# jean-pierreBoth/hnswlib-rs

Hardware: AMD Instinct MI355X
Metric: queries/sec (+ recall@10), batched HNSW search (higher is better)
Workload: dtype f32

## Files before the change

hnswlib-rs_amd/csrc/search_device.hip:

```cpp
#include <hip/hip_runtime.h>

#include <algorithm>
#include <chrono>
#include <cmath>
#include <cstdio>
#include <cstdlib>
#include <cstring>
#include <thread>
#include <vector>

#include "hnswio.hpp"
#include "search_device.hpp"
#include "search_kernels.hpp"
#include "worker_pool.hpp"

namespace hnswgpu {

namespace {
Knobs read_knobs() {
    Knobs k;
    auto num = [](const char* name, int unset) { const char* e = std::getenv(name); return e ? std::atoi(e) : unset; };
    auto flag = [](const char* name) { return std::getenv(name) != nullptr; };
    k.hash_bits = num("HNSWGPU_HASH_BITS", -1);
    k.no_sched = flag("HNSWGPU_NO_SCHED");
    k.no_pair_descent = flag("HNSWGPU_NO_PAIR_DESCENT");
    k.no_inkernel = flag("HNSWGPU_NO_INKERNEL");
    k.strict_wg_per_cu = num("HNSWGPU_STRICT_WG_PER_CU", -1);
    k.cand_lds = num("HNSWGPU_CAND_LDS", -1);
    k.waves_per_cu = num("HNSWGPU_WAVES_PER_CU", -1);
    k.exact_first = num("HNSWGPU_EXACT_FIRST", -1);
    k.trace_launch = flag("HNSWGPU_TRACE_LAUNCH");
    k.trace_host = flag("HNSWGPU_TRACE_HOST");
    k.host_threads = num("HNSWGPU_HOST_THREADS", -1);
    k.host_chunks = num("HNSWGPU_HOST_CHUNKS", -1);
    k.ffi_unpack = flag("HNSWGPU_FFI_UNPACK");
    k.pair_search = num("HNSWGPU_PAIR_SEARCH", -1);
    k.pair_tbits_delta = num("HNSWGPU_PAIR_TBITS_DELTA", 0);
    k.pair_wg_per_cu = num("HNSWGPU_PAIR_WG_PER_CU", -1);
    return k;
}
std::atomic<const Knobs*> g_knobs{nullptr};
}
const Knobs& knobs() {
    const Knobs* k = g_knobs.load(std::memory_order_acquire);
    if (k == nullptr) {
        const Knobs* fresh = new Knobs(read_knobs());
        if (g_knobs.compare_exchange_strong(k, fresh, std::memory_order_acq_rel)) k = fresh;
        else delete fresh;
    }
    return *k;
}
void reload_knobs() {
    g_knobs.store(new Knobs(read_knobs()), std::memory_order_release);
}

namespace {

#define HIP_TRY(expr)                                                                          \
    do {                                                                                       \
        hipError_t e_ = (expr);                                                                \
        if (e_ != hipSuccess) {                                                                \
            err = std::string(#expr) + ": " + hipGetErrorString(e_);                           \
            return ERR_DEVICE;                                                                 \
        }                                                                                      \
    } while (0)

hipError_t wait_stream(hipStream_t s) {
    const auto t0 = std::chrono::steady_clock::now();
    for (;;) {
        const hipError_t e = hipStreamQuery(s);
        if (e != hipErrorNotReady) return e;
        if (std::chrono::steady_clock::now() - t0 > std::chrono::milliseconds(20)) return hipStreamSynchronize(s);
    }
}
hipError_t wait_event(hipEvent_t ev) {
    const auto t0 = std::chrono::steady_clock::now();
    for (;;) {
        const hipError_t e = hipEventQuery(ev);
        if (e != hipErrorNotReady) return e;
        if (std::chrono::steady_clock::now() - t0 > std::chrono::milliseconds(20)) return hipEventSynchronize(ev);
    }
}

class DeviceGuard {
public:
    explicit DeviceGuard(int device) {
        if (device < 0) return;
        int cur = -1;
        if (hipGetDevice(&cur) != hipSuccess) cur = -1;
        if (cur == device) return;
        status_ = hipSetDevice(device);
        if (status_ == hipSuccess && cur >= 0) prev_ = cur;
    }
    ~DeviceGuard() { if (prev_ >= 0) (void)hipSetDevice(prev_); }
    DeviceGuard(const DeviceGuard&) = delete;
    DeviceGuard& operator=(const DeviceGuard&) = delete;
    hipError_t status() const { return status_; }
private:
    int prev_ = -1;
    hipError_t status_ = hipSuccess;
};

constexpr uint64_t PAIR_SEARCH_AUTO_MIN_QUERIES = 40000;
constexpr int STRICT_WG_PER_CU = 16;

uint32_t ceil_log2(uint64_t x) {
    uint32_t b = 0;
    while ((1ull << b) < x) ++b;
    return b;
}

const KernelSet& kernel_set(int metric) {
    switch (metric) {
        case DIST_L2: return kernels_for<DIST_L2>();
        case DIST_COSINE: return kernels_for<DIST_COSINE>();
        case DIST_DOT: return kernels_for<DIST_DOT>();
        case DIST_HELLINGER: return kernels_for<DIST_HELLINGER>();
        case DIST_JEFFREYS: return kernels_for<DIST_JEFFREYS>();
        case DIST_JENSENSHANNON: return kernels_for<DIST_JENSENSHANNON>();
        case KM_L2_SIMD8: return kernels_for<KM_L2_SIMD8>();
        case KM_COSINE_SIMD8: return kernels_for<KM_COSINE_SIMD8>();
        case KM_DOT_SIMD8: return kernels_for<KM_DOT_SIMD8>();
        case KM_L1_SIMD8: return kernels_for<KM_L1_SIMD8>();
        default: return kernels_for<DIST_L1>();
    }
}
// ... 50 lines not shown
    void free() {
        if (p) (void)hipHostFree(p);
        p = nullptr;
        dev = nullptr;
        cap = 0;
    }
};

void* pinned_alloc(size_t bytes, void** dev) {
    void* p = nullptr;
    if (hipHostMalloc(&p, bytes, hipHostMallocMapped | hipHostMallocPortable) != hipSuccess) { (void)hipGetLastError(); return nullptr; }
    if (hipHostGetDevicePointer(dev, p, 0) != hipSuccess) { (void)hipGetLastError(); (void)hipHostFree(p); return nullptr; }
    return p;
}
void pinned_free(void* p) {
    if (p) (void)hipHostFree(p);
}

struct DeviceIndex::Workspace {
    DevBuf qpad, tie, pre, order, retry[2], stats, bitmap, heaps, cand, oplog, allow, allowed_ids;
    PinnedBuf pin_in, pin_out;
    void* d_ctrl = nullptr;
    void* h_ctrl = nullptr;
    hipEvent_t ev_start = nullptr, ev_stop = nullptr, ev_ks = nullptr, ev_ke = nullptr;
    hipStream_t own_stream = nullptr;
    int init(std::string& err) {
        HIP_TRY(hipMalloc(&d_ctrl, 64));
        HIP_TRY(hipHostMalloc(&h_ctrl, 64, hipHostMallocDefault));
        HIP_TRY(hipEventCreate(&ev_start));
        HIP_TRY(hipEventCreate(&ev_stop));
        HIP_TRY(hipEventCreate(&ev_ks));
        HIP_TRY(hipEventCreate(&ev_ke));
        HIP_TRY(hipStreamCreateWithFlags(&own_stream, hipStreamNonBlocking));
        return OK;
    }
    ~Workspace() {
        for (DevBuf* b : {&qpad, &tie, &pre, &order, &retry[0], &retry[1], &stats, &bitmap, &heaps, &cand, &oplog, &allow, &allowed_ids})
            b->free();
        pin_in.free();
        pin_out.free();
        if (d_ctrl) (void)hipFree(d_ctrl);
        if (h_ctrl) (void)hipHostFree(h_ctrl);
        for (hipEvent_t e : {ev_start, ev_stop, ev_ks, ev_ke})
            if (e) (void)hipEventDestroy(e);
        if (own_stream) (void)hipStreamDestroy(own_stream);
    }
};

class DeviceIndex::Lease {
public:
    Lease(DeviceIndex* o, Workspace* w) : o_(o), w_(w) {}
    ~Lease() { if (w_) o_->release_ws(w_); }
    Lease(const Lease&) = delete;
    Lease& operator=(const Lease&) = delete;
    Workspace* get() const { return w_; }
private:
    DeviceIndex* o_;
    Workspace* w_;
};

DeviceIndex::Workspace* DeviceIndex::acquire(std::string& err) {
    {
        std::lock_guard<std::mutex> g(pool_mu_);
        if (!free_ws_.empty()) {
            Workspace* w = free_ws_.back();
// ... 132 lines not shown
CallInfo DeviceIndex::last_call() const {
    std::lock_guard<std::mutex> g(meta_mu_);
    return last_;
}

int DeviceIndex::upload(const FlatIndex& x, int device, std::string& err) {
    if (const char* e = std::getenv("HNSWGPU_STRICT_TIES")) strict_ties_.store(std::atoi(e) != 0);
    if (x.n == 0 || x.entry_flat == NO_POINT) { err = "cannot upload an empty index"; return ERR_EMPTY; }
    if (x.n >= 0x80000000ull) { err = "index too large for the device path (2^31 points or more)"; return ERR_ARG; }
    int ndev = 0;
    if (hipGetDeviceCount(&ndev) != hipSuccess || ndev == 0) { err = "no HIP device visible (a gfx950 GPU is required; there is no CPU fallback)"; return ERR_DEVICE; }
    if (device < 0 || device >= ndev) { err = "bad device ordinal"; return ERR_ARG; }
    release();
    DeviceGuard on_device(device);
    HIP_TRY(on_device.status());
    hipDeviceProp_t prop;
    HIP_TRY(hipGetDeviceProperties(&prop, device));
    num_cu_ = prop.multiProcessorCount;
    device_ = device;
    dist_ = x.dist;
    bytes_ = 0;
    descend_per_cu_[0].store(0);
    descend_per_cu_[1].store(0);

    const uint64_t n = x.n, d = x.dimension;
    DeviceIndexView v{};
    v.n = (uint32_t)n;
    v.d = (uint32_t)d;
    v.row_stride = (uint32_t)((d + 31) / 32 * 32);
    v.entry = x.entry_flat;
    v.entry_level = x.layer_of(x.entry_flat);
    v.search_layer = x.layer_to_search();
    for (unsigned l = 0; l <= NB_LAYER_MAX; ++l) v.layer_offset[l] = (uint32_t)x.layer_offset[l];

    {
        std::vector<float> pad((size_t)n * v.row_stride, 0.f);
        for (uint64_t f = 0; f < n; ++f) std::memcpy(pad.data() + f * v.row_stride, x.vectors.data() + f * d, d * sizeof(float));
        HIP_TRY(hipMalloc(&d_vec_, pad.size() * sizeof(float)));
        HIP_TRY(hipMemcpy(d_vec_, pad.data(), pad.size() * sizeof(float), hipMemcpyHostToDevice));
        bytes_ += pad.size() * sizeof(float);
    }
    {
        const unsigned sl = v.search_layer;
        uint64_t maxdeg = 1;
        for (uint64_t f = 0; f < n; ++f)
            maxdeg = std::max<uint64_t>(maxdeg, x.nbr_ptr[f * NB_LAYER_MAX + sl + 1] - x.nbr_ptr[f * NB_LAYER_MAX + sl]);
// ... 118 lines not shown
        a.id_stride = layout.id_stride;
        a.dist_stride = layout.dist_stride;
        a.count_stride = layout.count_stride;
        a.stats = stats;
        a.pre = w.pre.as<PreDescent>();
        x.heaps = w.heaps.as<hent_t>();
        x.heap_stride = heap_stride;
        x.cand_cap = (uint32_t)std::min<uint64_t>(cand_cap, 0xFFFFFFFFull);
        x.allow = d_allow;
        HIP_TRY(hipMemsetAsync(w.d_ctrl, 0, 16, stream));
        HIP_TRY(ks.launch_exact(ns, grid, lds, stream, v_, a, x));
        volatile uint32_t* ctrl = static_cast<volatile uint32_t*>(w.h_ctrl);
        HIP_TRY(hipMemcpyAsync(w.h_ctrl, w.d_ctrl, 16, hipMemcpyDeviceToHost, stream));
        HIP_TRY(wait_stream(stream));
        if (ctrl[1] != 0) { err = "internal error in the literal search kernel (a refused point inside return_points, or a candidate heap beyond every point)"; return ERR_DEVICE; }
        panics_total += ctrl[2];
        work = ctrl[3];
        qlist = w.retry[0].as<uint32_t>();
    }
    if (panics) *panics = panics_total;
    return OK;
}

int DeviceIndex::search_device(const float* d_queries, uint64_t nq, uint64_t d, uint64_t k, uint64_t ef_arg,
                               uint64_t* d_out_ids, float* d_out_dists, uint8_t* d_out_layer, int32_t* d_out_rank,
                               uint32_t* d_out_counts, uint32_t* d_stats, void* stream_v, const uint64_t* d_allowed,
                               uint64_t n_allowed, CallInfo* info_out, std::string& err, const RowFeed* feed, OutLayout layout) {
    if (!ready_) { err = "index is not resident on a device: call hnswgpu_upload first"; return ERR_DEVICE; }
    if (d != v_.d) { err = "query dimension differs from the index dimension"; return ERR_ARG; }
    CallInfo info{};
    auto publish = [&]() {
        if (info_out) *info_out = info;
        std::lock_guard<std::mutex> g(meta_mu_);
        last_ = info;
    };
    if (nq == 0) { publish(); return OK; }
    if (!d_queries || !d_out_ids || !d_out_dists || !d_out_counts) { err = "null buffer"; return ERR_ARG; }
    if (k == 0) { err = "knbn must be > 0"; return ERR_ARG; }
    const uint64_t ef = std::max(ef_arg, k);
    if (ef > 0x7FFFFFF0ull) { err = "ef too large"; return ERR_ARG; }
    if (nq > 0xFFFFFFF0ull) { err = "too many queries in one batch"; return ERR_ARG; }
    const bool filtered = d_allowed != nullptr || n_allowed != 0;
    hipStream_t stream = static_cast<hipStream_t>(stream_v);
    DeviceGuard on_device(device_);
    HIP_TRY(on_device.status());
    Lease lease(this, acquire(err));
    if (!lease.get()) return ERR_DEVICE;
    Workspace& w = *lease.get();
    struct DrainOnError {
        hipStream_t s;
        bool done = false;
        ~DrainOnError() { if (!done) (void)hipStreamSynchronize(s); }
    } drain{stream};

    HIP_TRY(w.qpad.ensure(nq * v_.row_stride * sizeof(float)));
    if (!d_stats) HIP_TRY(w.stats.ensure(nq * 8 * sizeof(uint32_t)));
    uint32_t* stats = d_stats ? d_stats : w.stats.as<uint32_t>();
    const bool strict_ties = strict_ties_.load();

    HIP_TRY(w.pre.ensure(nq * sizeof(PreDescent)));
    const uint32_t tile_bytes = tile_bytes_for(kernel_metric(), v_.row_stride);
    {
        const KernelSet& ks = kernel_set(kernel_metric());
        const bool pair = up_deg_max_ <= 16u && kernel_metric() < KM_SIMD8_FIRST && !knobs().no_pair_descent;
        const size_t descend_lds = (pair ? 2u : 1u) * (size_t)tile_bytes + IDS_BYTES;
        int per_cu = descend_per_cu_[pair].load();
        if (per_cu <= 0) {
            HIP_TRY(ks.descend_occupancy(descend_lds, pair, &per_cu));
            per_cu = std::max(1, per_cu);
            descend_per_cu_[pair].store(per_cu);
        }
        const uint64_t chunk = feed ? std::max<uint64_t>(1, feed->chunk_rows) : nq;
        for (uint64_t lo = 0; lo < nq; lo += chunk) {
            const uint64_t hi = std::min(nq, lo + chunk);
            if (feed) feed->fill(feed->ctx, lo, hi);
            DescendArgs da{};
            da.src = d_queries + lo * v_.d;
            da.qpad = w.qpad.as<float>() + lo * v_.row_stride;
            da.pre = w.pre.as<PreDescent>() + lo;
            da.nq = (uint32_t)(hi - lo);
            da.tile_bytes = tile_bytes;
            da.nrm2 = static_cast<const double*>(d_nrm2_);
            da.ctrl = lo == 0 ? static_cast<uint32_t*>(w.d_ctrl) : nullptr;
            da.ctrl_words = 16;
            da.pair = pair ? 1u : 0u;
            const uint64_t waves = pair ? (hi - lo + 1) / 2 : hi - lo;
            HIP_TRY(ks.launch_descend((uint32_t)std::min<uint64_t>(waves, (uint64_t)per_cu * (uint64_t)num_cu_), stream, v_, da,
                                      LaunchEvents{lo == 0 ? w.ev_start : nullptr, nullptr}));
        }
    }

    if (filtered || ef > 1024) {
        const uint32_t* d_allow = nullptr;
        if (filtered) {
            HIP_TRY(w.allow.ensure((uint64_t)((v_.n + 31) / 32) * sizeof(uint32_t)));
            HIP_TRY(launch_allow_bitmap(stream, v_.origin_id, v_.n, d_allowed, n_allowed, w.allow.as<uint32_t>()));
            d_allow = w.allow.as<uint32_t>();
        }
        HIP_TRY(hipEventRecord(w.ev_ks, stream));
        int rc = run_exact(w, w.qpad.as<float>(), nullptr, (uint32_t)nq, k, ef, d_allow, d_out_ids, d_out_dists, d_out_layer, d_out_rank,
                           d_out_counts, stats, stream, &info.panics, err, layout);
        if (rc != OK) return rc;
        HIP_TRY(hipEventRecord(w.ev_stop, stream));
        HIP_TRY(wait_event(w.ev_stop));
        float ms = 0.f, ms_main = 0.f;
        HIP_TRY(hipEventElapsedTime(&ms, w.ev_start, w.ev_stop));
        HIP_TRY(hipEventElapsedTime(&ms_main, w.ev_ks, w.ev_stop));
        info.ms = ms;
        info.main_ms = ms_main;
        info.launches = 1;
        publish();
        drain.done = true;
        return OK;
    }

    HIP_TRY(w.tie.ensure(nq * sizeof(uint32_t)));
    HIP_TRY(w.retry[0].ensure(nq * sizeof(uint32_t)));
    HIP_TRY(w.retry[1].ensure(nq * sizeof(uint32_t)));

    int slots = 1;
    while ((uint64_t)slots * 64 < ef) slots *= 2;
    if (slots == 8) slots = 16;
    if (v_.deg_stride > 64u) slots = 16;

    const uint32_t idbits = std::max<uint32_t>(1u, ceil_log2(v_.n));
    const uint64_t expect = ef * std::min<uint64_t>(v_.deg_stride, 64);
    uint32_t tbits = std::min<uint32_t>(14u, std::max<uint32_t>(8u, ceil_log2(expect)));
    {
        std::lock_guard<std::mutex> g(meta_mu_);
        if (adapt_ef_ == ef && adapt_tbits_ != 0) tbits = adapt_tbits_;
    }
    bool env_forced = false;
    const Knobs& kn = knobs();
    if (kn.hash_bits >= 6 && kn.hash_bits <= 14) { tbits = (uint32_t)kn.hash_bits; env_forced = true; }
    const uint32_t tbits_first = tbits;
    const size_t lds_fixed = tile_bytes + IDS_BYTES;
    int table = TABLE_LDS_CELL16;
    bool grown = false;

    const bool scheduled = nq >= 256 && !kn.no_sched;
    if (scheduled) {
        HIP_TRY(w.order.ensure(nq * sizeof(uint32_t)));
        HIP_TRY(kernel_set(kernel_metric()).launch_order(stream, w.pre.as<PreDescent>(), (uint32_t)nq, w.order.as<uint32_t>()));
    }
    uint32_t launches = 0, stop_recorded_after = ~0u;
    uint32_t work = (uint32_t)nq;
    uint32_t n_flagged = 0, n_literal = 0;
    const uint32_t* qlist = scheduled ? w.order.as<uint32_t>() : nullptr;
    int pingpong = 0;
    bool all_done = false;
    const bool pair_auto = (kernel_metric() == DIST_COSINE || kernel_metric() == DIST_DOT) && v_.row_stride <= 32u && strict_ties &&
                           nq >= PAIR_SEARCH_AUTO_MIN_QUERIES;
    if (kn.pair_search > 0 || (kn.pair_search < 0 && pair_auto)) {
        const int tbp = (int)tbits + kn.pair_tbits_delta;
        const uint32_t tb = (uint32_t)std::max(6, std::min<int>(tbp, (int)std::min(14u, idbits + 3u)));
        const bool ok = ef <= 128 && v_.deg_stride <= 64u && kernel_metric() < KM_SIMD8_FIRST && nq >= 512 && idbits >= tb - 3u && idbits - (tb - 3u) <= 13u &&
                        idbits - (tb - 3u) >= 1u;
        if (ok) {
            const KernelSet& ks = kernel_set(kernel_metric());
            SearchArgs a{};
            a.tbits = tb;
            a.restbits = idbits - (tb - 3u);
            a.idbits = idbits;
            a.tile_bytes = tile_bytes;
            a.nrm2 = static_cast<const double*>(d_nrm2_);
            const size_t lds = pair_lds_bytes(tile_bytes, tb, (uint32_t)ef);
            int per_cu = 0;
            HIP_TRY(ks.pair_occupancy(lds, &per_cu));
            if (per_cu >= 1) {
                if (kn.pair_wg_per_cu > 0) per_cu = std::min(per_cu, kn.pair_wg_per_cu);
                const uint64_t npairs = (nq + 1) / 2;
                const uint32_t grid = (uint32_t)std::min<uint64_t>((uint64_t)per_cu * (uint64_t)num_cu_, npairs);
                if (kn.trace_launch)
                    std::fprintf(stderr, "[hnswgpu launch] pair pass: %u queries, %d workgroups per CU, %zu bytes of LDS each, tables 2^%u cells\n",
                                 work, per_cu, lds, tb);
                a.queries = w.qpad.as<float>();
                a.qlist = qlist;
                a.nq = work;
                a.k = (uint32_t)k;
                a.ef = (uint32_t)ef;
                a.work_counter = static_cast<uint32_t*>(w.d_ctrl);
                a.overflow_count = static_cast<uint32_t*>(w.d_ctrl) + 1;
                a.retry_out = w.retry[pingpong].as<uint32_t>();
                a.out_ids = d_out_ids;
                a.out_dists = d_out_dists;
                a.out_layer = d_out_layer;
                a.out_rank = d_out_rank;
                a.out_counts = d_out_counts;
                a.id_stride = layout.id_stride;
                a.dist_stride = layout.dist_stride;
                a.count_stride = layout.count_stride;
                a.stats = stats;
                a.pre = w.pre.as<PreDescent>();
                a.tie_list = w.tie.as<uint32_t>();
                a.pair_ties_to_retry = strict_ties ? 1u : 0u;
                {
                    a.bitmap_words = (v_.n + 31) / 32;
                    const uint64_t slice = (uint64_t)a.bitmap_words * sizeof(uint32_t);
                    const uint64_t blocks = std::min<uint64_t>(2ull * grid, std::max<uint64_t>(2, (4ull << 30) / slice));
// ... 41 lines not shown
                table = TABLE_LDS_CELL32;
                lds += (size_t)4 << tb;
            }
            a.tbits = tb;
        }
        a.tile_bytes = tile_bytes;
        a.nrm2 = static_cast<const double*>(d_nrm2_);
        a.idbits = idbits;
        const KernelSet& ks = kernel_set(kernel_metric());
        const bool strict_kernel = strict_ties && table != TABLE_GLOBAL_BITMAP && !kn.no_inkernel;
        if (slots <= (strict_kernel ? HNSW_MERGE_SMAX : HNSW_MERGE_LEAN_SMAX)) {
            a.merge_entries = (uint32_t)slots * 64u + 64u;
            lds += (size_t)a.merge_entries * sizeof(hent_t);
        }
        int per_cu = 0;
        int strict_cap = STRICT_WG_PER_CU;
        if (kn.strict_wg_per_cu > 0) strict_cap = kn.strict_wg_per_cu;
        if (strict_kernel) {
            a.cand_lds = 256;
            if (kn.cand_lds >= 0) {
                a.cand_lds = (uint32_t)std::min(4096, kn.cand_lds);
            } else {
                int occ256 = 0, occ512 = 0;
                HIP_TRY(ks.occupancy(slots, table, true, lds + 256 * sizeof(hent_t), &occ256));
                HIP_TRY(ks.occupancy(slots, table, true, lds + 512 * sizeof(hent_t), &occ512));
                if (std::min(occ512, strict_cap) >= std::min(occ256, strict_cap)) a.cand_lds = 512;
            }
            lds += (size_t)a.cand_lds * sizeof(hent_t);
        }
        HIP_TRY(ks.occupancy(slots, table, strict_kernel, lds, &per_cu));
        if (per_cu < 1) per_cu = 1;
        if (strict_kernel) per_cu = std::min(per_cu, strict_cap);
        if (kn.waves_per_cu > 0) per_cu = std::max(1, std::min(per_cu, kn.waves_per_cu));
        uint32_t grid = (uint32_t)std::min<uint64_t>((uint64_t)per_cu * (uint64_t)num_cu_, work);
        if (kn.trace_launch)
            std::fprintf(stderr, "[hnswgpu launch] %u queries, %d workgroups per CU (strict cap %d), %zu bytes of LDS each (literal heap: %u entries), table 2^%u cells, strict %d, work list %s, slots %d, visited set %s\n",
                         work, per_cu, strict_cap, lds, a.cand_lds, a.tbits, (int)strict_kernel,
                         qlist ? "sorted" : "input order", slots,
                         table == TABLE_LDS_CELL16 ? "cell16" : table == TABLE_LDS_CELL32 ? "cell32" : "bitmap");
        a.queries = w.qpad.as<float>();
        a.qlist = qlist;
        a.nq = work;
        a.k = (uint32_t)k;
        a.ef = (uint32_t)ef;
        a.work_counter = static_cast<uint32_t*>(w.d_ctrl);
        a.overflow_count = static_cast<uint32_t*>(w.d_ctrl) + 1;
        a.retry_out = w.retry[pingpong].as<uint32_t>();
        a.out_ids = d_out_ids;
        a.out_dists = d_out_dists;
        a.out_layer = d_out_layer;
        a.out_rank = d_out_rank;
        a.out_counts = d_out_counts;
        a.id_stride = layout.id_stride;
        a.dist_stride = layout.dist_stride;
        a.count_stride = layout.count_stride;
        a.stats = stats;
        a.pre = w.pre.as<PreDescent>();
        {
            a.bitmap_words = (v_.n + 31) / 32;
            const uint64_t slice = (uint64_t)a.bitmap_words * sizeof(uint32_t);
            uint64_t blocks = std::min<uint64_t>(grid, std::max<uint64_t>(1, (4ull << 30) / slice));
            if (table == TABLE_GLOBAL_BITMAP) grid = (uint32_t)blocks;
            HIP_TRY(w.bitmap.ensure(blocks * slice));
            a.bitmap = w.bitmap.as<uint32_t>();
            a.bitmap_blocks = (uint32_t)blocks;
        }
        a.tie_list = w.tie.as<uint32_t>();
        if (strict_kernel) {
            const uint32_t cap = 4096;
            const uint64_t need = (uint64_t)grid * cap * sizeof(hent_t);
            HIP_TRY(w.cand.ensure(need));
            HIP_TRY(w.oplog.ensure(need));
            a.cand_scratch = w.cand.as<hent_t>();
            a.cand_cap = cap;
            a.oplog = w.oplog.as<hent_t>();
            a.oplog_cap = cap;
            if (kn.exact_first >= 0) a.exact_first = kn.exact_first != 0 ? 1u : 0u;
        }
        if (launches != 0) HIP_TRY(hipMemsetAsync(w.d_ctrl, 0, 16, stream));
        HIP_TRY(ks.launch_search(slots, table, strict_kernel, grid, lds, stream, v_, a,
                                 launches == 0 ? LaunchEvents{w.ev_ks, w.ev_ke} : LaunchEvents{}));
        ++launches;
        volatile uint32_t* ctrl = static_cast<volatile uint32_t*>(w.h_ctrl);
        HIP_TRY(hipMemcpyAsync(w.h_ctrl, w.d_ctrl, 24, hipMemcpyDeviceToHost, stream));
        HIP_TRY(hipEventRecord(w.ev_stop, stream));
        stop_recorded_after = launches;
        HIP_TRY(wait_stream(stream));
        n_flagged = ctrl[4];
        n_literal += ctrl[5];
        if (launches == 1 && table != TABLE_GLOBAL_BITMAP && !env_forced && nq >= 256) {
            uint32_t next = tbits_first;
            if ((uint64_t)ctrl[2] * 8 > nq && tbits_first < 14u) next = tbits_first + 1;
            else if ((uint64_t)ctrl[3] * 32 < nq && tbits_first > 8u) next = tbits_first - 1;
            std::lock_guard<std::mutex> g(meta_mu_);
            adapt_ef_ = ef;
            adapt_tbits_ = next;
        }
        if (ctrl[1] == 0) break;
        work = ctrl[1];
        qlist = w.retry[pingpong].as<uint32_t>();
        pingpong ^= 1;
        if (table == TABLE_GLOBAL_BITMAP) { err = "internal error: bitmap visited set reported an overflow"; return ERR_DEVICE; }
        if (!grown && tbits < 14u) {
            tbits = std::min<uint32_t>(14u, tbits + 2u);
            grown = true;
        } else {
            table = TABLE_GLOBAL_BITMAP;
        }
    }
    info.ties = n_flagged + n_literal;
    if (strict_ties && n_flagged > 0) {
        int rc = run_exact(w, w.qpad.as<float>(), w.tie.as<uint32_t>(), n_flagged, k, ef, nullptr, d_out_ids, d_out_dists, d_out_layer,
                           d_out_rank, d_out_counts, stats, stream, nullptr, err, layout);
        if (rc != OK) return rc;
        ++launches;
    }
    if (stop_recorded_after != launches) {
        HIP_TRY(hipEventRecord(w.ev_stop, stream));
        HIP_TRY(wait_event(w.ev_stop));
    }
    float ms = 0.f, ms_main = 0.f;
    HIP_TRY(hipEventElapsedTime(&ms, w.ev_start, w.ev_stop));
    HIP_TRY(hipEventElapsedTime(&ms_main, w.ev_ks, w.ev_ke));
    info.ms = ms;
    info.main_ms = ms_main;
    info.launches = launches;
    publish();
    drain.done = true;
    return OK;
}

namespace {
struct HostCall {
    const float* queries;
    const float* const* rows;
    float* hq;
    uint64_t d, nq, chunk_rows, task_rows, tasks_per_chunk, n_chunks;
    std::atomic<uint64_t> next_gather{0};
    std::vector<std::atomic<uint32_t>> chunk_left;
    std::atomic<int> phase{0};
    std::atomic<uint64_t> next_unpack{0};
    uint64_t unpack_rows = 256;
    DeviceIndex::HostAnswers answers{};
    const uint32_t* stats = nullptr;
    uint8_t* flags = nullptr;
// ... 496 lines not shown
```

hnswlib-rs_amd/csrc/search_device.hpp:

```cpp
#pragma once
#include <atomic>
#include <cstdint>
#include <memory>
#include <mutex>
#include <string>
#include <vector>
#include "builder.hpp"
#include "flat_index.hpp"

namespace hnswgpu {

constexpr int ARITH_SCALAR = 0, ARITH_SIMD8 = 1;

struct Knobs {
    int hash_bits = -1;
    bool no_sched = false;
    bool no_pair_descent = false;
    bool no_inkernel = false;
    int strict_wg_per_cu = -1;
    int cand_lds = -1;
    int waves_per_cu = -1;
    int exact_first = -1;
    bool trace_launch = false;
    bool trace_host = false;
    int host_threads = -1;
    int host_chunks = -1;
    bool ffi_unpack = false;
    int pair_search = -1;
    int pair_tbits_delta = 0;
    int pair_wg_per_cu = -1;
};
const Knobs& knobs();
void reload_knobs();

struct DeviceIndexView {
    const float* vec;
    const uint32_t* nbr0;
    const uint32_t* up_ptr;
    const uint32_t* up_ids;
    const uint64_t* origin_id;
    uint32_t n;
    uint32_t d;
    uint32_t row_stride;
    uint32_t deg_stride;
    uint32_t n_up_layers;
    uint32_t entry;
    uint32_t entry_level;
    uint32_t search_layer;
    uint32_t layer_offset[NB_LAYER_MAX + 1];
};

struct CallInfo {
    double ms = 0.0;
// ... 90 lines not shown
    bool ready_ = false;
    int device_ = -1;
    int dist_ = DIST_L2;
    int num_cu_ = 0;
    uint64_t bytes_ = 0;
    void* d_vec_ = nullptr;
    void* d_nbr0_ = nullptr;
    void* d_up_ptr_ = nullptr;
    void* d_up_ids_ = nullptr;
    void* d_origin_ = nullptr;
    void* d_nrm2_ = nullptr;
    std::mutex pool_mu_;
    std::vector<std::unique_ptr<Workspace>> all_ws_;
    std::vector<Workspace*> free_ws_;
    mutable std::mutex meta_mu_;
    uint64_t adapt_ef_ = 0;
    uint32_t adapt_tbits_ = 0;
    CallInfo last_{};
    std::atomic<bool> strict_ties_{true};
    std::atomic<int> arith_{0};
    int kernel_metric() const;
    std::atomic<int> descend_per_cu_[2] = {{0}, {0}};
    uint32_t up_deg_max_ = 0;
    mutable std::mutex ext_mu_;
    mutable std::shared_ptr<void> ext_;
};

int device_count();
int gather_sharded_answers(const int* devices, int n_shards, const uint64_t* nq_shard, uint64_t k, const uint64_t* const* d_ids,
                           const float* const* d_dists, const uint8_t* const* d_layer, const int32_t* const* d_rank,
                           const uint32_t* const* d_counts, int root_device, uint64_t* root_ids, float* root_dists,
                           uint8_t* root_layer, int32_t* root_rank, uint32_t* root_counts, void* root_stream, std::string& err);
std::unique_ptr<BuildSearchBackend> make_device_build_backend(int device);
int eval_distance_matrix_device(int dist, const float* queries, uint64_t nq, const float* rows, uint64_t n, uint64_t d,
                                uint32_t nf, bool pairs, float* out, std::string& err, int arithmetic = 0);

int lane_lab_device(int device, uint32_t mode, uint32_t p0, uint32_t p1, uint32_t p2, const uint32_t* ops, uint32_t n_ops,
                    const uint32_t* lanes, uint32_t n_lane_sets, uint32_t* out, uint32_t out_words, std::string& err);

}
```

hnswlib-rs_amd/csrc/search_kernels.hpp:

```cpp
#pragma once
#include <hip/hip_runtime.h>
#include <hip/hip_ext.h>
#include <cstdint>
#include "search_device.hpp"

namespace hnswgpu {

constexpr uint32_t EXPANDED = 0x80000000u;
constexpr uint32_t EMPTY_SLOT = 0xFFFFFFFFu;
constexpr int TABLE_LDS_CELL16 = 0;
constexpr int TABLE_LDS_CELL32 = 1;
constexpr int TABLE_GLOBAL_BITMAP = 2;

constexpr int KM_SIMD8_FIRST = 7;
constexpr int KM_L2_SIMD8 = 7, KM_COSINE_SIMD8 = 8, KM_DOT_SIMD8 = 9, KM_L1_SIMD8 = 10;
constexpr int KM_COUNT = 11;
inline int simd8_kernel_metric(int dist) {
    return dist == DIST_L2 ? KM_L2_SIMD8 : dist == DIST_COSINE ? KM_COSINE_SIMD8 : dist == DIST_DOT ? KM_DOT_SIMD8 : dist == DIST_L1 ? KM_L1_SIMD8 : -1;
}

constexpr uint32_t IDS_BYTES = 64 * 4;

typedef unsigned long long hent_t;

// ... 29 lines not shown
    uint32_t* overflow_count;
    uint32_t* retry_out;
    uint32_t* bitmap;
    uint32_t bitmap_words;
    uint32_t bitmap_blocks;
    uint32_t* tie_list;
    hent_t* cand_scratch;
    uint32_t cand_cap;
    uint32_t cand_lds;
    uint32_t merge_entries;
    uint32_t exact_first;
    uint32_t pair_ties_to_retry;
    hent_t* oplog;
    uint32_t oplog_cap;
    const double* nrm2;
    uint64_t* out_ids;
    float* out_dists;
    uint8_t* out_layer;
    int32_t* out_rank;
    uint32_t* out_counts;
    const PreDescent* pre;
    uint32_t* stats;
    uint32_t id_stride, dist_stride, count_stride;
};

struct ExactArgs {
    hent_t* heaps;
    uint64_t heap_stride;
    uint32_t cand_cap;
    uint32_t r_lds_cap;
    uint32_t cand_lds;
    const uint32_t* allow;
};

struct BuildLists {
    uint32_t* lists[NB_LAYER_MAX];
    uint32_t stride[NB_LAYER_MAX];
};
struct BuildArgs {
    const float* vec;
    uint32_t row_stride;
    const uint32_t* lists[NB_LAYER_MAX];
    uint32_t stride[NB_LAYER_MAX];
    const uint8_t* level;
    const uint32_t* slot0;
    uint32_t first, count;
// ... 103 lines not shown
```

hnswlib-rs_amd/csrc/search_kernels.inc:

```
#pragma clang fp contract(off)
#include <type_traits>
#include "ln_f32.hpp"

#ifndef HNSW_LB_WAVES
#define HNSW_LB_WAVES 5
#endif
#ifndef HNSW_MERGE_LISTS
#define HNSW_MERGE_LISTS 1
#endif
#ifndef HNSW_LB_WAVES_STRICT
#define HNSW_LB_WAVES_STRICT 4
#endif
#ifndef HNSW_LB_DESCEND
#define HNSW_LB_DESCEND 6
#endif
#ifndef HNSW_DPP_ASM
#define HNSW_DPP_ASM 1
#endif
#ifndef HNSW_PIPE_ROWS
#define HNSW_PIPE_ROWS 1
#endif
#ifndef HNSW_DEEP_G2
#define HNSW_DEEP_G2 1
#endif
// ... 1036 lines not shown
                best_id = readlane_u(id, ctz64(eq));
            }
        }
        if (best < dcur) {
            dcur = best;
            pivot = best_id;
        }
    }
}

template <int METRIC>
__global__ __launch_bounds__(64, HNSW_LB_DESCEND) void hnsw_descend_kernel(DeviceIndexView ix, DescendArgs a) {
    extern __shared__ __attribute__((aligned(16))) unsigned char lds_raw[];
    float4* tile = reinterpret_cast<float4*>(lds_raw);
    uint32_t* ids_lds = reinterpret_cast<uint32_t*>(lds_raw + a.tile_bytes);
    const int lane = (int)threadIdx.x;
    if (blockIdx.x == 0 && a.ctrl != nullptr && (uint32_t)lane < a.ctrl_words) a.ctrl[lane] = 0u;
    const uint32_t row_stride = ix.row_stride, d = ix.d;
    for (uint32_t q = blockIdx.x; q < a.nq; q += gridDim.x) {
        const float* __restrict__ src = a.src + (size_t)q * d;
        float* tf = reinterpret_cast<float*>(tile);
        for (uint32_t c = (uint32_t)lane; c < row_stride; c += 64) tf[c] = c < d ? src[c] : 0.f;
        __syncthreads();
        float4* dst = reinterpret_cast<float4*>(a.qpad + (size_t)q * row_stride);
        for (uint32_t i = (uint32_t)lane; i < (row_stride >> 2); i += 64) dst[i] = tile[i];
        finish_staged_query<METRIC>(tile, row_stride, lane, d);
        uint32_t pivot, n_dist = 0, n_expand = 0, n_ids = 0;
        float dcur;
        greedy_descent<METRIC>(ix, (nrm_ptr_t)a.nrm2, tile, ids_lds, lane, pivot, dcur, n_dist, n_expand, n_ids);
        if (lane == 0) a.pre[q] = PreDescent{pivot, __float_as_uint(dcur), n_dist, n_expand};
        __syncthreads();
    }
}

template <int METRIC>
__global__ __launch_bounds__(64, HNSW_LB_DESCEND) void hnsw_descend_pair_kernel(DeviceIndexView ix, DescendArgs a) {
    if constexpr (METRIC < KM_SIMD8_FIRST) {
        extern __shared__ __attribute__((aligned(16))) unsigned char lds_raw[];
        const int lane = (int)threadIdx.x;
        const uint32_t half = (uint32_t)lane >> 5, hl = (uint32_t)lane & 31u;
        float4* tile = reinterpret_cast<float4*>(lds_raw + (size_t)half * a.tile_bytes);
        uint32_t* ids_lds = reinterpret_cast<uint32_t*>(lds_raw + 2u * (size_t)a.tile_bytes);
        if (blockIdx.x == 0 && a.ctrl != nullptr && (uint32_t)lane < a.ctrl_words) a.ctrl[lane] = 0u;
        const uint32_t row_stride = ix.row_stride, d = ix.d, nchunk = row_stride >> 2;
        const nrm_ptr_t nrm2 = (nrm_ptr_t)a.nrm2;
        const uint32_t npair = (a.nq + 1u) >> 1;
        for (uint32_t p = blockIdx.x; p < npair; p += gridDim.x) {
            const uint32_t q = 2u * p + half < a.nq ? 2u * p + half : 2u * p;
            const bool mine = 2u * p + half < a.nq;
            uint32_t pivot = ix.entry;
            uint32_t pb = 0, pe = 0;
            const int top = (int)ix.entry_level;
            if (top >= 1 && (uint32_t)top <= ix.n_up_layers) {
                const uint32_t* ptr = ix.up_ptr + (size_t)(top - 1) * ((size_t)ix.n + 1);
                pb = ptr[pivot];
                pe = ptr[pivot + 1];
            }
            const uint32_t id_next = hl < pe - pb ? ix.up_ids[pb + hl] : pivot;
            const float* __restrict__ src = a.src + (size_t)q * d;
            float* tf = reinterpret_cast<float*>(tile);
            for (uint32_t c = hl; c < row_stride; c += 32) tf[c] = c < d ? src[c] : 0.f;
            __syncthreads();
            float4* dst = reinterpret_cast<float4*>(a.qpad + (size_t)q * row_stride);
            for (uint32_t i = hl; i < nchunk; i += 32) dst[i] = tile[i];
            if constexpr (METRIC == DIST_COSINE) {
                double s1 = 0.;
                for (uint32_t c = 0; c < nchunk; ++c) {
                    const float4 v = tile[c];
                    s1 = s1 + (double)(v.x * v.x); s1 = s1 + (double)(v.y * v.y); s1 = s1 + (double)(v.z * v.z); s1 = s1 + (double)(v.w * v.w);
                }
                if (hl == 0u) *reinterpret_cast<double*>(tile + nchunk) = s1;
            }
            const uint32_t rhalf = ((uint32_t)lane >> 4) & 1u, rj = (uint32_t)lane & 15u;
            float dcur = INFINITY;
            bool have_dcur = false;
            if (top < 1 || readlane_u(pe - pb, 0) > 15u) {
                if ((uint32_t)lane < 32u) ids_lds[lane] = pivot;
                __syncthreads();
                const float res0 = group_dist<METRIC, 2>(ix.vec, row_stride, nrm2, tile, ids_lds, 0u, 32u, lane, INFINITY, NoOverlap(), false);
                const float e_a = readlane_f(res0, 0), e_b = readlane_f(res0, 16);
                dcur = half != 0u ? e_b : e_a;
                have_dcur = true;
            }
            __syncthreads();
            uint32_t n_dist = 1, n_expand = 0;
            for (int layer = top; layer >= 1; --layer) {
                const uint32_t len = pe - pb;
// ... 378 lines not shown
    const int lane = (int)threadIdx.x;
    const uint32_t words = ka->a.bitmap_words, restbits = ka->a.restbits, idbits = ka->a.idbits;
    uint32_t* bitmap = ka->a.bitmap + (size_t)blockIdx.x * words;
    const uint32_t* table = reinterpret_cast<const uint32_t*>(lds_raw + ka->a.tile_bytes + IDS_BYTES);
    const uint32_t table_cells = 1u << ka->a.tbits;
    for (uint32_t i = (uint32_t)lane; i < words; i += 64) bitmap[i] = 0u;
    __syncthreads();
    for (uint32_t i = (uint32_t)lane; i < table_cells; i += 64) {
        uint32_t id = EMPTY_SLOT;
        if constexpr (TABLE == TABLE_LDS_CELL16) {
            const uint32_t half = (table[i >> 1] >> ((i & 1u) * 16u)) & 0xFFFFu;
            if (half != 0u) {
                const uint32_t bdisp = (half & 0x7FFFu) >> restbits;
                const uint32_t rest = half & ((1u << restbits) - 1u);
                const uint32_t home = ((i >> 3) - bdisp) & ((table_cells >> 3) - 1u);
                id = unmix_id((home << restbits) | rest, idbits);
            }
        } else if constexpr (TABLE == TABLE_LDS_CELL32) {
            id = table[i];
        }
        if (id != EMPTY_SLOT) atomicOr(&bitmap[id >> 5], 1u << (id & 31u));
    }
    __syncthreads();
}

template <int S>
__device__ __forceinline__ bool final_order_ambiguous(const float (&rd)[S], uint32_t len, uint32_t k, float taint_w, int lane) {
    const uint32_t kk = k < len ? k : len;
    if (kk == 0u) return false;
    unsigned long long bad = 0ull;
#pragma unroll
    for (int s = 0; s < S; ++s) {
        const uint32_t j = (uint32_t)s * 64u + (uint32_t)lane;
        const float nxt = __shfl_down(rd[s], 1);
        const float edge = s + 1 < S ? r_dist_at<S>(rd, (uint32_t)(s + 1) * 64u) : INFINITY;
        const float nd = lane == 63 ? edge : nxt;
        bad |= __ballot(j < kk && j + 1u < len && rd[s] == nd);
    }
    return bad != 0ull || r_dist_at<S>(rd, kk - 1u) == taint_w;
}

template <int METRIC, int S, int TABLE, bool STRICT>
__global__ __launch_bounds__(64, STRICT ? (S >= 16 ? 2 : S == 4 && HNSW_PIPE_ROWS != 0 ? 3 : HNSW_LB_WAVES_STRICT) : (S >= 16 ? 4 : HNSW_LB_WAVES)) void hnsw_search_kernel(DeviceIndexView ix, SearchArgs a) {
    extern __shared__ __attribute__((aligned(16))) unsigned char lds_raw[];
    const void* const kargs = (const void*)__builtin_amdgcn_kernarg_segment_ptr();
    float4* tile = reinterpret_cast<float4*>(lds_raw);
// ... 332 lines not shown
                    }
                    out_status = 3;
                }
            }
        } else {
            if (status == 0 && tie_any && !flag_tie && final_order_ambiguous<S>(rd, len, a.k, taint_w, lane)) flag_tie = true;
        }
        if (status == 0 && flag_tie) status = 2;
        {
            QueryEnd<S> e;
#pragma unroll
            for (int s = 0; s < S; ++s) { e.rd[s] = rd[s]; e.ri[s] = ri[s]; }
            e.q = q; e.len = len; e.status = status; e.out_status = out_status;
            e.n_dist = n_dist; e.n_expand = n_expand; e.n_ids = n_ids; e.t_start = t_start;
            e.flags = (tie_any ? 1u : 0u) | (literal_used ? 2u : 0u) | (use_bm ? 4u : 0u);
            e.feedback = (use_bm ? 1u : 0u) | (n_visited > (table_limit >> 1) ? 2u : 0u) | (TABLE != TABLE_GLOBAL_BITMAP ? 4u : 0u);
#if HNSW_PHASE_TIMING
            e.ph[0] = ph[0]; e.ph[1] = ph[1]; e.ph[2] = ph[2]; e.ph[3] = ph[3]; e.ph_miss = ph_miss;
#endif
            finish_query<S>(kargs, e);
        }
        __syncthreads();
    }
}


template <int METRIC, int NS>
__global__ __launch_bounds__(64, 4) void hnsw_search_exact_kernel(DeviceIndexView ix, SearchArgs a, ExactArgs x) {
    RegHeap<(NS > 0 ? NS : 1)> RR;
    extern __shared__ __attribute__((aligned(16))) unsigned char lds_raw[];
    float4* tile = reinterpret_cast<float4*>(lds_raw);
    uint32_t* ids_lds = reinterpret_cast<uint32_t*>(lds_raw + a.tile_bytes);
    const int lane = (int)threadIdx.x;
    uint32_t* bitmap = a.bitmap + (size_t)blockIdx.x * a.bitmap_words;
    const nrm_ptr_t nrm2 = (nrm_ptr_t)a.nrm2;
    hent_t* lds_heaps = reinterpret_cast<hent_t*>(lds_raw + a.tile_bytes + IDS_BYTES);
    hent_t* glb = x.heaps + (size_t)blockIdx.x * x.heap_stride;
    const uint32_t r_lds = a.ef + 2u <= x.r_lds_cap ? a.ef + 2u : x.r_lds_cap;
    const HeapMem R{lds_heaps, glb, r_lds};
    const HeapMem Cq{lds_heaps + r_lds, glb + (a.ef + 2u), x.cand_lds};
    const bool filtered = x.allow != nullptr;
    auto allowed = [&](uint32_t flat) __attribute__((always_inline)) -> bool { return (x.allow[flat >> 5] >> (flat & 31u)) & 1u; };
    auto r_push_capped = [&](uint32_t& len, hent_t item) __attribute__((always_inline)) {
        if constexpr (NS > 0) {
            if (len == RegHeap<(NS > 0 ? NS : 1)>::CAP) { RR.push_then_pop_full(item, lane); return; }
            RR.push(len, item, lane);
// ... 523 lines not shown
```

Before: 9.434 million.

## Signal search completion via mapped-memory exit ticket and skip query padding copy

The last workgroup to finish the search kernel, found by an atomic ticket, writes the control counters tagged with a sequence number into coherent mapped host memory. The host spin-polls that memory instead of issuing a memcpy, an event record and a stream wait, which is meant to cut end-of-launch latency. Queries are also read directly when they are already aligned and unpadded, skipping the copy into a padded buffer. Occupancy queries are cached per configuration. The cost is more complex synchronisation, plus host spinning with a fallback to stream sync.

```diff
diff --git a/hnswlib-rs_amd/csrc/search_device.hip b/hnswlib-rs_amd/csrc/search_device.hip
--- a/hnswlib-rs_amd/csrc/search_device.hip
+++ b/hnswlib-rs_amd/csrc/search_device.hip
@@ -37,6 +37,8 @@
     k.pair_search = num("HNSWGPU_PAIR_SEARCH", -1);
     k.pair_tbits_delta = num("HNSWGPU_PAIR_TBITS_DELTA", 0);
     k.pair_wg_per_cu = num("HNSWGPU_PAIR_WG_PER_CU", -1);
+    k.no_exit_ticket = flag("HNSWGPU_NO_EXIT_TICKET");
+    k.no_direct_queries = flag("HNSWGPU_NO_DIRECT_QUERIES");
     return k;
 }
 std::atomic<const Knobs*> g_knobs{nullptr};
@@ -79,6 +81,28 @@
         const hipError_t e = hipEventQuery(ev);
         if (e != hipErrorNotReady) return e;
         if (std::chrono::steady_clock::now() - t0 > std::chrono::milliseconds(20)) return hipEventSynchronize(ev);
+    }
+}
+
+hipError_t wait_done(const void* h_done, uint32_t seq, hipStream_t s, uint32_t (&ctrl)[6]) {
+    const volatile uint64_t* slot = static_cast<const volatile uint64_t*>(h_done);
+    auto arrived = [&]() {
+        for (int i = 0; i < 6; ++i) {
+            const uint64_t v = slot[i];
+            if ((uint32_t)(v >> 32) != seq) return false;
+            ctrl[i] = (uint32_t)v;
+        }
+        return true;
+    };
+    const auto t0 = std::chrono::steady_clock::now();
+    for (;;) {
+        if (arrived()) { std::atomic_thread_fence(std::memory_order_acquire); return hipSuccess; }
+        __builtin_ia32_pause();
+        if (std::chrono::steady_clock::now() - t0 > std::chrono::milliseconds(20)) {
+            const hipError_t e = hipStreamSynchronize(s);
+            if (e != hipSuccess) return e;
+            return arrived() ? hipSuccess : hipErrorUnknown;
+        }
     }
 }
 
@@ -102,6 +126,7 @@
 };
 
 constexpr uint64_t PAIR_SEARCH_AUTO_MIN_QUERIES = 40000;
+constexpr uint32_t CTRL_BYTES = 256, TICKET_WORD = 32;
 constexpr int STRICT_WG_PER_CU = 16;
 
 uint32_t ceil_log2(uint64_t x) {
@@ -198,11 +223,17 @@
     PinnedBuf pin_in, pin_out;
     void* d_ctrl = nullptr;
     void* h_ctrl = nullptr;
+    void* h_done = nullptr;
+    void* d_done = nullptr;
+    uint32_t done_seq = 0;
     hipEvent_t ev_start = nullptr, ev_stop = nullptr, ev_ks = nullptr, ev_ke = nullptr;
     hipStream_t own_stream = nullptr;
     int init(std::string& err) {
-        HIP_TRY(hipMalloc(&d_ctrl, 64));
+        HIP_TRY(hipMalloc(&d_ctrl, CTRL_BYTES));
         HIP_TRY(hipHostMalloc(&h_ctrl, 64, hipHostMallocDefault));
+        HIP_TRY(hipHostMalloc(&h_done, 64, hipHostMallocMapped | hipHostMallocPortable | hipHostMallocCoherent));
+        std::memset(h_done, 0, 64);
+        HIP_TRY(hipHostGetDevicePointer(&d_done, h_done, 0));
         HIP_TRY(hipEventCreate(&ev_start));
         HIP_TRY(hipEventCreate(&ev_stop));
         HIP_TRY(hipEventCreate(&ev_ks));
@@ -217,6 +248,7 @@
         pin_out.free();
         if (d_ctrl) (void)hipFree(d_ctrl);
         if (h_ctrl) (void)hipHostFree(h_ctrl);
+        if (h_done) (void)hipHostFree(h_done);
         for (hipEvent_t e : {ev_start, ev_stop, ev_ks, ev_ke})
             if (e) (void)hipEventDestroy(e);
         if (own_stream) (void)hipStreamDestroy(own_stream);
@@ -395,6 +427,10 @@
     bytes_ = 0;
     descend_per_cu_[0].store(0);
     descend_per_cu_[1].store(0);
+    {
+        std::lock_guard<std::mutex> g(occ_mu_);
+        occ_.clear();
+    }
 
     const uint64_t n = x.n, d = x.dimension;
     DeviceIndexView v{};
@@ -559,6 +595,20 @@
     return OK;
 }
 
+int DeviceIndex::search_occupancy(int metric, int slots, int table, bool strict, size_t lds, int* per_cu) {
+    const uint64_t key = ((uint64_t)metric << 56) | ((uint64_t)slots << 48) | ((uint64_t)table << 44) | ((uint64_t)strict << 40) | (uint64_t)lds;
+    {
+        std::lock_guard<std::mutex> g(occ_mu_);
+        for (const auto& e : occ_)
+            if (e.first == key) { *per_cu = e.second; return (int)hipSuccess; }
+    }
+    const hipError_t e = kernel_set(metric).occupancy(slots, table, strict, lds, per_cu);
+    if (e != hipSuccess) return (int)e;
+    std::lock_guard<std::mutex> g(occ_mu_);
+    occ_.emplace_back(key, *per_cu);
+    return (int)hipSuccess;
+}
+
 int DeviceIndex::search_device(const float* d_queries, uint64_t nq, uint64_t d, uint64_t k, uint64_t ef_arg,
                                uint64_t* d_out_ids, float* d_out_dists, uint8_t* d_out_layer, int32_t* d_out_rank,
                                uint32_t* d_out_counts, uint32_t* d_stats, void* stream_v, const uint64_t* d_allowed,
@@ -590,7 +640,10 @@
         ~DrainOnError() { if (!done) (void)hipStreamSynchronize(s); }
     } drain{stream};
 
-    HIP_TRY(w.qpad.ensure(nq * v_.row_stride * sizeof(float)));
+    const bool direct_queries = feed == nullptr && v_.d == v_.row_stride && (reinterpret_cast<uintptr_t>(d_queries) & 15u) == 0u &&
+                                !knobs().no_direct_queries;
+    if (!direct_queries) HIP_TRY(w.qpad.ensure(nq * v_.row_stride * sizeof(float)));
+    const float* const qrows = direct_queries ? d_queries : w.qpad.as<float>();
     if (!d_stats) HIP_TRY(w.stats.ensure(nq * 8 * sizeof(uint32_t)));
     uint32_t* stats = d_stats ? d_stats : w.stats.as<uint32_t>();
     const bool strict_ties = strict_ties_.load();
@@ -613,13 +666,13 @@
             if (feed) feed->fill(feed->ctx, lo, hi);
             DescendArgs da{};
             da.src = d_queries + lo * v_.d;
-            da.qpad = w.qpad.as<float>() + lo * v_.row_stride;
+            da.qpad = direct_queries ? nullptr : w.qpad.as<float>() + lo * v_.row_stride;
             da.pre = w.pre.as<PreDescent>() + lo;
             da.nq = (uint32_t)(hi - lo);
             da.tile_bytes = tile_bytes;
             da.nrm2 = static_cast<const double*>(d_nrm2_);
             da.ctrl = lo == 0 ? static_cast<uint32_t*>(w.d_ctrl) : nullptr;
-            da.ctrl_words = 16;
+            da.ctrl_words = knobs().no_exit_ticket ? 16 : TICKET_WORD + 1;
             da.pair = pair ? 1u : 0u;
             const uint64_t waves = pair ? (hi - lo + 1) / 2 : hi - lo;
             HIP_TRY(ks.launch_descend((uint32_t)std::min<uint64_t>(waves, (uint64_t)per_cu * (uint64_t)num_cu_), stream, v_, da,
@@ -635,7 +688,7 @@
             d_allow = w.allow.as<uint32_t>();
         }
         HIP_TRY(hipEventRecord(w.ev_ks, stream));
-        int rc = run_exact(w, w.qpad.as<float>(), nullptr, (uint32_t)nq, k, ef, d_allow, d_out_ids, d_out_dists, d_out_layer, d_out_rank,
+        int rc = run_exact(w, qrows, nullptr, (uint32_t)nq, k, ef, d_allow, d_out_ids, d_out_dists, d_out_layer, d_out_rank,
                            d_out_counts, stats, stream, &info.panics, err, layout);
         if (rc != OK) return rc;
         HIP_TRY(hipEventRecord(w.ev_stop, stream));
@@ -681,6 +734,7 @@
         HIP_TRY(kernel_set(kernel_metric()).launch_order(stream, w.pre.as<PreDescent>(), (uint32_t)nq, w.order.as<uint32_t>()));
     }
     uint32_t launches = 0, stop_recorded_after = ~0u;
+    bool ended_by_ticket = false;
     uint32_t work = (uint32_t)nq;
     uint32_t n_flagged = 0, n_literal = 0;
     const uint32_t* qlist = scheduled ? w.order.as<uint32_t>() : nullptr;
@@ -711,7 +765,7 @@
                 if (kn.trace_launch)
                     std::fprintf(stderr, "[hnswgpu launch] pair pass: %u queries, %d workgroups per CU, %zu bytes of LDS each, tables 2^%u cells\n",
                                  work, per_cu, lds, tb);
-                a.queries = w.qpad.as<float>();
+                a.queries = qrows;
                 a.qlist = qlist;
                 a.nq = work;
                 a.k = (uint32_t)k;
@@ -799,13 +853,13 @@
                 a.cand_lds = (uint32_t)std::min(4096, kn.cand_lds);
             } else {
                 int occ256 = 0, occ512 = 0;
-                HIP_TRY(ks.occupancy(slots, table, true, lds + 256 * sizeof(hent_t), &occ256));
-                HIP_TRY(ks.occupancy(slots, table, true, lds + 512 * sizeof(hent_t), &occ512));
+                HIP_TRY((hipError_t)search_occupancy(kernel_metric(), slots, table, true, lds + 256 * sizeof(hent_t), &occ256));
+                HIP_TRY((hipError_t)search_occupancy(kernel_metric(), slots, table, true, lds + 512 * sizeof(hent_t), &occ512));
                 if (std::min(occ512, strict_cap) >= std::min(occ256, strict_cap)) a.cand_lds = 512;
             }
             lds += (size_t)a.cand_lds * sizeof(hent_t);
         }
-        HIP_TRY(ks.occupancy(slots, table, strict_kernel, lds, &per_cu));
+        HIP_TRY((hipError_t)search_occupancy(kernel_metric(), slots, table, strict_kernel, lds, &per_cu));
         if (per_cu < 1) per_cu = 1;
         if (strict_kernel) per_cu = std::min(per_cu, strict_cap);
         if (kn.waves_per_cu > 0) per_cu = std::max(1, std::min(per_cu, kn.waves_per_cu));
@@ -815,7 +869,7 @@
                          work, per_cu, strict_cap, lds, a.cand_lds, a.tbits, (int)strict_kernel,
                          qlist ? "sorted" : "input order", slots,
                          table == TABLE_LDS_CELL16 ? "cell16" : table == TABLE_LDS_CELL32 ? "cell32" : "bitmap");
-        a.queries = w.qpad.as<float>();
+        a.queries = qrows;
         a.qlist = qlist;
         a.nq = work;
         a.k = (uint32_t)k;
@@ -855,14 +909,30 @@
             if (kn.exact_first >= 0) a.exact_first = kn.exact_first != 0 ? 1u : 0u;
         }
         if (launches != 0) HIP_TRY(hipMemsetAsync(w.d_ctrl, 0, 16, stream));
+        const bool ticketed = launches == 0 && !kn.no_exit_ticket;
+        uint32_t seq = 0;
+        if (ticketed) {
+            if (++w.done_seq == 0u) ++w.done_seq;
+            seq = w.done_seq;
+            a.exit_ticket = static_cast<uint32_t*>(w.d_ctrl) + TICKET_WORD;
+            a.done_slot = static_cast<unsigned long long*>(w.d_done);
+            a.done_seq = seq;
+        }
         HIP_TRY(ks.launch_search(slots, table, strict_kernel, grid, lds, stream, v_, a,
                                  launches == 0 ? LaunchEvents{w.ev_ks, w.ev_ke} : LaunchEvents{}));
         ++launches;
-        volatile uint32_t* ctrl = static_cast<volatile uint32_t*>(w.h_ctrl);
-        HIP_TRY(hipMemcpyAsync(w.h_ctrl, w.d_ctrl, 24, hipMemcpyDeviceToHost, stream));
-        HIP_TRY(hipEventRecord(w.ev_stop, stream));
-        stop_recorded_after = launches;
-        HIP_TRY(wait_stream(stream));
+        uint32_t ctrl[6];
+        if (ticketed) {
+            HIP_TRY(wait_done(w.h_done, seq, stream, ctrl));
+            ended_by_ticket = true;
+        } else {
+            const volatile uint32_t* h = static_cast<const volatile uint32_t*>(w.h_ctrl);
+            HIP_TRY(hipMemcpyAsync(w.h_ctrl, w.d_ctrl, 24, hipMemcpyDeviceToHost, stream));
+            HIP_TRY(hipEventRecord(w.ev_stop, stream));
+            stop_recorded_after = launches;
+            HIP_TRY(wait_stream(stream));
+            for (int i = 0; i < 6; ++i) ctrl[i] = h[i];
+        }
         n_flagged = ctrl[4];
         n_literal += ctrl[5];
         if (launches == 1 && table != TABLE_GLOBAL_BITMAP && !env_forced && nq >= 256) {
@@ -887,17 +957,20 @@
     }
     info.ties = n_flagged + n_literal;
     if (strict_ties && n_flagged > 0) {
-        int rc = run_exact(w, w.qpad.as<float>(), w.tie.as<uint32_t>(), n_flagged, k, ef, nullptr, d_out_ids, d_out_dists, d_out_layer,
+        int rc = run_exact(w, qrows, w.tie.as<uint32_t>(), n_flagged, k, ef, nullptr, d_out_ids, d_out_dists, d_out_layer,
                            d_out_rank, d_out_counts, stats, stream, nullptr, err, layout);
         if (rc != OK) return rc;
         ++launches;
     }
-    if (stop_recorded_after != launches) {
+    const bool one_launch = ended_by_ticket && launches == 1;
+    if (one_launch) {
+        HIP_TRY(wait_event(w.ev_ke));
+    } else if (stop_recorded_after != launches) {
         HIP_TRY(hipEventRecord(w.ev_stop, stream));
         HIP_TRY(wait_event(w.ev_stop));
     }
     float ms = 0.f, ms_main = 0.f;
-    HIP_TRY(hipEventElapsedTime(&ms, w.ev_start, w.ev_stop));
+    HIP_TRY(hipEventElapsedTime(&ms, w.ev_start, one_launch ? w.ev_ke : w.ev_stop));
     HIP_TRY(hipEventElapsedTime(&ms_main, w.ev_ks, w.ev_ke));
     info.ms = ms;
     info.main_ms = ms_main;
diff --git a/hnswlib-rs_amd/csrc/search_device.hpp b/hnswlib-rs_amd/csrc/search_device.hpp
--- a/hnswlib-rs_amd/csrc/search_device.hpp
+++ b/hnswlib-rs_amd/csrc/search_device.hpp
@@ -4,6 +4,7 @@
 #include <memory>
 #include <mutex>
 #include <string>
+#include <utility>
 #include <vector>
 #include "builder.hpp"
 #include "flat_index.hpp"
@@ -29,6 +30,8 @@
     int pair_search = -1;
     int pair_tbits_delta = 0;
     int pair_wg_per_cu = -1;
+    bool no_exit_ticket = false;
+    bool no_direct_queries = false;
 };
 const Knobs& knobs();
 void reload_knobs();
@@ -165,6 +168,9 @@
     int kernel_metric() const;
     std::atomic<int> descend_per_cu_[2] = {{0}, {0}};
     uint32_t up_deg_max_ = 0;
+    int search_occupancy(int metric, int slots, int table, bool strict, size_t lds, int* per_cu);
+    std::mutex occ_mu_;
+    std::vector<std::pair<uint64_t, int>> occ_;
     mutable std::mutex ext_mu_;
     mutable std::shared_ptr<void> ext_;
 };
diff --git a/hnswlib-rs_amd/csrc/search_kernels.hpp b/hnswlib-rs_amd/csrc/search_kernels.hpp
--- a/hnswlib-rs_amd/csrc/search_kernels.hpp
+++ b/hnswlib-rs_amd/csrc/search_kernels.hpp
@@ -75,6 +75,9 @@
     const PreDescent* pre;
     uint32_t* stats;
     uint32_t id_stride, dist_stride, count_stride;
+    uint32_t* exit_ticket;
+    unsigned long long* done_slot;
+    uint32_t done_seq;
 };
 
 struct ExactArgs {
diff --git a/hnswlib-rs_amd/csrc/search_kernels.inc b/hnswlib-rs_amd/csrc/search_kernels.inc
--- a/hnswlib-rs_amd/csrc/search_kernels.inc
+++ b/hnswlib-rs_amd/csrc/search_kernels.inc
@@ -1082,8 +1082,10 @@
         float* tf = reinterpret_cast<float*>(tile);
         for (uint32_t c = (uint32_t)lane; c < row_stride; c += 64) tf[c] = c < d ? src[c] : 0.f;
         __syncthreads();
-        float4* dst = reinterpret_cast<float4*>(a.qpad + (size_t)q * row_stride);
-        for (uint32_t i = (uint32_t)lane; i < (row_stride >> 2); i += 64) dst[i] = tile[i];
+        if (a.qpad != nullptr) {
+            float4* dst = reinterpret_cast<float4*>(a.qpad + (size_t)q * row_stride);
+            for (uint32_t i = (uint32_t)lane; i < (row_stride >> 2); i += 64) dst[i] = tile[i];
+        }
         finish_staged_query<METRIC>(tile, row_stride, lane, d);
         uint32_t pivot, n_dist = 0, n_expand = 0, n_ids = 0;
         float dcur;
@@ -1121,8 +1123,10 @@
             float* tf = reinterpret_cast<float*>(tile);
             for (uint32_t c = hl; c < row_stride; c += 32) tf[c] = c < d ? src[c] : 0.f;
             __syncthreads();
-            float4* dst = reinterpret_cast<float4*>(a.qpad + (size_t)q * row_stride);
-            for (uint32_t i = hl; i < nchunk; i += 32) dst[i] = tile[i];
+            if (a.qpad != nullptr) {
+                float4* dst = reinterpret_cast<float4*>(a.qpad + (size_t)q * row_stride);
+                for (uint32_t i = hl; i < nchunk; i += 32) dst[i] = tile[i];
+            }
             if constexpr (METRIC == DIST_COSINE) {
                 double s1 = 0.;
                 for (uint32_t c = 0; c < nchunk; ++c) {
@@ -1547,6 +1551,23 @@
         if (id != EMPTY_SLOT) atomicOr(&bitmap[id >> 5], 1u << (id & 31u));
     }
     __syncthreads();
+}
+
+__device__ __attribute__((noinline, unused)) void leave_launch(const void* kargs) {
+    const kernargs_t ka = uniform_kernargs(kargs);
+    uint32_t* const ticket = ka->a.exit_ticket;
+    if (ticket == nullptr || threadIdx.x != 0) return;
+    asm volatile("s_waitcnt vmcnt(0)" ::: "memory");
+    const uint32_t drawn = __hip_atomic_fetch_add(ticket, 1u, __ATOMIC_RELAXED, __HIP_MEMORY_SCOPE_AGENT);
+    if (drawn + 1u != gridDim.x) return;
+    uint32_t* const ctrl = ka->a.work_counter;
+    unsigned long long* const slot = ka->a.done_slot;
+    const unsigned long long seq = (unsigned long long)ka->a.done_seq << 32;
+    uint32_t c[6];
+#pragma unroll
+    for (int i = 0; i < 6; ++i) c[i] = __hip_atomic_load(ctrl + i, __ATOMIC_ACQUIRE, __HIP_MEMORY_SCOPE_AGENT);
+#pragma unroll
+    for (int i = 0; i < 6; ++i) __hip_atomic_store(slot + i, seq | c[i], __ATOMIC_RELAXED, __HIP_MEMORY_SCOPE_SYSTEM);
 }
 
 template <int S>
@@ -1925,6 +1946,7 @@
         }
         __syncthreads();
     }
+    leave_launch(kargs);
 }
 
 
```

Measured after the change: 9.394 million. Within noise of the previous version (-0.4%).
